# pangsu0613/TransCAR

Hardware: AMD Instinct MI355X
Metric: nuScenes frames/sec (6-cam+radar, 900 queries): fusion decoder (Detr3DHead.forward + box decode), FPN features resident in HBM (higher is better)
Workload: dtype f32 (linear steps and attention core of the batched launches: f16x2 split operands, 3 v_mfma_f32_16x16x32_f16 products, fp32 accumulate; activations of the 32-row tiles held as two f16 planes; 4- / 8-row tiles: f32 MFMA)

## Files before the change

### include/transcar_hip.h

```cpp
#ifndef TRANSCAR_HIP_H
#define TRANSCAR_HIP_H

#include <stddef.h>

#ifdef __cplusplus
extern "C" {
#endif

#define TC_MAX_LEVELS 4
#define TC_MAX_LAYERS 8
#define TC_MAX_RADAR_LAYERS 3
#define TC_MAX_CAM_LOGITS 256
#define TC_ABI_VERSION 13

typedef void* tc_stream_t;

typedef struct { const float* w; const float* b; } tc_linear;
typedef struct { const float* g; const float* b; } tc_lnorm;
typedef struct { tc_linear l0; tc_lnorm n1; tc_linear l3; tc_lnorm n4; } tc_pos_encoder;
typedef struct { tc_linear l0; tc_lnorm n1; tc_linear l3; tc_lnorm n4; tc_linear l6; } tc_cls_branch;
typedef struct { tc_linear l0; tc_linear l2; tc_linear l4; } tc_reg_branch;
typedef struct { tc_linear in_proj; tc_linear out_proj; } tc_mha;

typedef struct {
// ... 196 lines not shown
                       int num_classes, int code_size, int max_num,
                       const float* post_center_range ,
                       float* boxes, float* scores, int* labels, unsigned char* valid,
                       void* workspace, size_t workspace_bytes, tc_stream_t stream);
int tc_box_decode_kept(const float* cls_scores, const float* bbox_preds, int B, int Q, int num_classes,
                       int code_size, int max_num, const float* post_center_range ,
                       float score_threshold, int use_threshold, int z_shift,
                       float* kept_boxes, float* kept_scores, long long* kept_labels, int* kept_count,
                       tc_stream_t stream);

size_t tc_head_workspace_bytes(const tc_head_weights* w, int B, int T);
size_t tc_cam_pregather_workspace_bytes(const tc_head_weights* w, int B);
size_t tc_head_packed_bytes(const tc_head_weights* w);
int tc_head_pack_weights(const tc_head_weights* w, void* packed, size_t packed_bytes,
                         tc_head_weights* packed_view, tc_stream_t stream);
int tc_head_repack_trainable(const tc_head_weights* w, tc_head_weights* packed_view,
                             tc_stream_t stream);
int tc_head_repack_trainable_ex(const tc_head_weights* w, tc_head_weights* packed_view, int copies,
                                tc_stream_t stream);
int tc_head_forward(const tc_head_weights* w, const tc_head_weights* packed_view,
                    const tc_feats_nhwc* feats, int B,
                    const float* lidar2img , float img_h, float img_w,
                    const float* radar_tokens, int T, int pad_mult,
                    float* all_cls_scores, float* all_bbox_preds,
                    const tc_head_aux* aux ,
                    const tc_head_options* options ,
                    void* workspace, size_t workspace_bytes, tc_stream_t stream);



// ... 117 lines not shown
```

### transcar_amd/_lib.py

```python
import ctypes as C
import os

_HERE = os.path.dirname(os.path.abspath(__file__))
LIB_PATH = os.environ.get('TRANSCAR_HIP_LIB') or os.path.join(_HERE, 'lib', 'libtranscar_hip.so')

TC_MAX_LEVELS = 4
TC_MAX_LAYERS = 8
TC_MAX_RADAR_LAYERS = 3
TC_ABI_VERSION = 13

c_fp = C.c_void_p


class TransCARHipError(RuntimeError):
    pass


TC_MAX_CAM_LOGITS = 256


def check_num_points(num_points, num_cams, num_levels):
    if int(num_points) < 1 or num_cams * num_levels * int(num_points) > TC_MAX_CAM_LOGITS:
        raise TransCARHipError(
            'Detr3DCrossAtten(HIP): num_points=%r is not supported (num_points >= 1 and '
# ... 145 lines not shown
    'tc_radar_gated_xattn_fwd': (_i, [_P(tc_mha), _vp, _vp, _vp, _i, _vp, _vp,
                                      _i, _i, _i, _i, _i, _i, _f, _f, _vp,
                                      _vp, _vp, _sz, _vp]),
    'tc_radar_fusion_fwd': (_i, [_P(tc_head_weights), _vp, _vp, _vp, _vp, _i, _i, _i, _i, _i,
                                 _vp, _vp, _vp, _P(tc_head_options), _vp, _sz, _vp]),
    'tc_box_decode_workspace_bytes': (_sz, [_i, _i, _i]),
    'tc_box_decode_topk': (_i, [_vp, _vp, _i, _i, _i, _i, _i, _P(_f), _vp,
                                _vp, _vp, _vp, _vp, _sz, _vp]),
    'tc_box_decode_kept': (_i, [_vp, _vp, _i, _i, _i, _i, _i, _P(_f), _f, _i, _i, _vp, _vp, _vp, _vp, _vp]),
    'tc_head_workspace_bytes': (_sz, [_P(tc_head_weights), _i, _i]),
    'tc_cam_pregather_workspace_bytes': (_sz, [_P(tc_head_weights), _i]),
    'tc_head_packed_bytes': (_sz, [_P(tc_head_weights)]),
    'tc_head_pack_weights': (_i, [_P(tc_head_weights), _vp, _sz,
                                  _P(tc_head_weights), _vp]),
    'tc_head_repack_trainable': (_i, [_P(tc_head_weights), _P(tc_head_weights), _vp]),
    'tc_head_forward': (_i, [_P(tc_head_weights), _P(tc_head_weights),
                             _P(tc_feats_nhwc), _i, _vp,
                             _f, _f, _vp, _i, _i, _vp, _vp, _P(tc_head_aux),
                             _P(tc_head_options), _vp, _sz, _vp]),
    'tc_linear_gated_fwd': (_i, [_vp, _vp, _vp, _vp, _vp, _vp, _i, _i, _i, _vp]),
    'tc_linear_bwd_data': (_i, [_vp, _vp, _vp, _vp, _vp, _vp, _i, _i, _i, _f,
                                _i, _vp]),
    'tc_linear_bwd_weight': (_i, [_vp, _vp, _vp, _vp, _vp, _vp, _i, _i, _i, _f,
                                  _vp]),
    'tc_add_layernorm_bwd': (_i, [_vp, _vp, _vp, _vp, _vp, _vp, _vp, _vp, _i,
                                  _i, _vp]),
    'tc_radar_reference_l1': (_i, [_vp, _P(_f), _vp, _vp, _i, _vp]),
    'tc_box_add_ref_fwd': (_i, [_vp, _i, _vp, _i, _vp, _i, _vp, _i, _vp]),
    'tc_box_add_ref_bwd': (_i, [_vp, _i, _vp, _i, _vp]),
    'tc_radar_attn_core_fwd': (_i, [_vp, _f, _vp, _vp, _i, _vp, _i, _vp, _i,
# ... 79 lines not shown
```

### transcar_amd/csrc/chain.hip

```cpp
#include <stdlib.h>
#include <string.h>

#include <type_traits>

#include "kernels.hpp"
#ifdef TC_CHAIN_STAMPS
__device__ long long g_cam_stamps[4][8];
#define CAM_STAMP(slot)                                                                        \
  do {                                                                                         \
    if (blockIdx.x == 100 && (threadIdx.x & 63) == 0)                                          \
      g_cam_stamps[(threadIdx.x >> 6) & 3][(slot)] = __builtin_amdgcn_s_memtime();             \
  } while (0)
#endif
#include "rowdev.hpp"
#define TC_ONCE_LD(p) ldg4_stream(p)
#ifdef TC_CHAIN_DUMP
__device__ float* g_chain_dump;
__device__ long long g_chain_dump_floats;
#endif

namespace tc {

namespace {

// ... 63 lines not shown
enum Flags : short {
  F_GATE = 1,
  F_SCALEQ = 2,
  F_WOFF = 4,
  F_LN_RELU = 8,
  F_SKIP_NONEXT = 16,
  F_WAVE1 = 32,
  F_NOT_W0 = 64,
  F_LN_XP = 128,
  F_IFHIT = 256,
  F_GPRE = 512,
  F_CMASK = 1024,
  F_CMASK_SCALE = 2048,
  F_CARRY = 4096,
  F_NOT_LAYER0 = 8192,
  F_PRESYNC = 16384
};
enum GSel : short {
  G_NONE = -1, G_HS = 0, G_QK, G_VT, G_INITREF, G_ATTN_O, G_XIN, G_POS, G_CLS, G_KV0, G_KV1, G_KV2,
  G_QF, G_RFEAT, G_COUNT
};

struct StepDesc {
  short kind, wp, wp2, K, N, src, src2, dst, res, act, flags, gsel, gtsel, sync;
};
constexpr StepDesc PROG_DECODER_T[] = {
    {K_LOAD, 0, 0, 0, 0, B_NONE, B_NONE, B_U1, B_NONE, 0, 0, G_ATTN_O, G_NONE, 0},
    {K_LOAD, 0, 0, 0, 0, B_NONE, B_NONE, B_X, B_NONE, 0, 0, G_XIN, G_NONE, 1},
    {K_LINEAR, 1, -1, 256, 256, B_U1, B_NONE, B_U2, B_X, 0, 0, G_NONE, G_NONE, 1},
    {K_LN, 2, -1, 0, 0, B_U2, B_NONE, B_X, B_U1, 0, F_LN_XP, G_NONE, G_NONE, 1},
    {K_LINEAR, 3, -1, 256, N_LOGITS, B_U1, B_NONE, B_L, B_NONE, 0, 0, G_NONE, G_NONE, 0},
    {K_POSENC, 5, 6, 0, 0, B_NONE, B_NONE, B_U2, B_NONE, 0, F_NOT_W0, G_NONE, G_NONE, 1},
    {K_SAMPLE, 0, 0, 0, 0, B_L, B_NONE, B_U3, B_NONE, 0, 0, G_NONE, G_NONE, 1},
    {K_LINEAR, 7, -1, 256, 256, B_U2, B_NONE, B_U1, B_NONE, 0, 0, G_NONE, G_NONE, 1},
    {K_LINEAR, 4, -1, 256, 256, B_U3, B_NONE, B_U2, B_X, 0, 0, G_NONE, G_NONE, 1},
    {K_LN, 9, 8, 0, 0, B_U2, B_U1, B_X, B_NONE, 0, 0, G_NONE, G_NONE, 1},
    {K_LINEAR, 10, -1, 256, 512, B_X, B_NONE, B_A, B_NONE, 1, 0, G_NONE, G_NONE, 1},
    {K_LINEAR, 11, -1, 512, 256, B_A, B_NONE, B_U3, B_X, 0, 0, G_NONE, G_NONE, 1},
    {K_LN, 12, -1, 0, 0, B_U3, B_NONE, B_X, B_U1, 0, F_LN_XP, G_HS, G_NONE, 1},
    {K_LINEAR, 13, -1, 256, 256, B_X, B_NONE, B_U2, B_NONE, 1, 0, G_NONE, G_NONE, 0},
    {K_LINEAR, 16, -1, 256, 512, B_U1, B_NONE, B_NONE, B_NONE, 0, F_SCALEQ | F_SKIP_NONEXT, G_QK, G_NONE, 0},
    {K_LINEAR, 16, -1, 256, 256, B_X, B_NONE, B_NONE, B_NONE, 0, F_WOFF | F_SKIP_NONEXT, G_NONE, G_VT, 1},
    {K_LINEAR, 14, -1, 256, 256, B_U2, B_NONE, B_U3, B_NONE, 1, 0, G_NONE, G_NONE, 0},
    {K_NARROW, 15, -1, 256, N_CODE, B_U3, B_U1, B_L, B_NONE, 0, F_PRESYNC, G_NONE, G_NONE, 1},
    {K_REFUPD, 0, 0, 0, 0, B_L, B_NONE, B_NONE, B_NONE, 0, 0, G_NONE, G_NONE, 0},
    {K_END, 0, 0, 0, 0, 0, 0, 0, 0, 0, 0, 0, 0, 0}};
constexpr StepDesc PROG_PROLOGUE_T[] = {
    {K_LOAD, 0, 0, 0, 0, B_NONE, B_NONE, B_U1, B_NONE, 0, 0, G_POS, G_NONE, 0},
    {K_LOAD, 0, 0, 0, 0, B_NONE, B_NONE, B_X, B_NONE, 0, 0, G_XIN, G_NONE, 1},
    {K_LINEAR, 0, -1, 256, 3, B_U1, B_NONE, B_NONE, B_NONE, 2, 0, G_INITREF, G_NONE, 0},
    {K_LINEAR, 16, -1, 256, 512, B_X, B_U1, B_NONE, B_NONE, 0, F_SCALEQ, G_QK, G_NONE, 0},
    {K_LINEAR, 16, -1, 256, 256, B_X, B_NONE, B_NONE, B_NONE, 0, F_WOFF, G_NONE, G_VT, 0},
    {K_END, 0, 0, 0, 0, 0, 0, 0, 0, 0, 0, 0, 0, 0}};
constexpr StepDesc PROG_RADAR_ENC_T[] = {
    {K_TOKENS, 0, 0, 0, 0, B_NONE, B_NONE, B_A, B_NONE, 0, 0, G_NONE, G_NONE, 1},
    {K_POSENC, 0, 1, 0, 0, B_A, B_NONE, B_U3, B_NONE, 0, 0, G_NONE, G_NONE, 0},
    {K_LINEAR, 4, -1, 36, 64, B_A, B_NONE, B_X, B_NONE, 1, 0, G_NONE, G_NONE, 1},
    {K_LINEAR, 2, -1, 256, 256, B_U3, B_NONE, B_U1, B_NONE, 0, 0, G_NONE, G_NONE, 0},
    {K_LINEAR, 5, -1, 64, 128, B_X, B_NONE, B_U2, B_NONE, 1, 0, G_NONE, G_NONE, 1},
    {K_LINEAR, 6, -1, 128, 256, B_U2, B_NONE, B_X, B_NONE, 1, 0, G_NONE, G_NONE, 1},
    {K_LN, 3, -1, 0, 0, B_U1, B_NONE, B_U2, B_X, 0, F_LN_RELU, G_NONE, G_NONE, 1},
// ... 90 lines not shown
  int last_cls_only;
  const float* ref_in; int ref_mod; float* ref_out; float* box_m;
  CamK cam; unsigned long long* pair_counter;
  const float* pre; const int* premask;
  const float* tokens; int RI, T, pad_mult;
  const float* ref_last; const float* box_in;
  int cen_from_box;
  float rmin[TC_MAX_RADAR_LAYERS], rmax[TC_MAX_RADAR_LAYERS];
  float* all_box; int* hits;
  const int* row_perm;
  float* tape[T_COUNT]; size_t tape_stride; size_t hits_stride;
  DropK rdrop;
  const float* bwd_cxy[TC_MAX_RADAR_LAYERS]; int bwd_ldc[TC_MAX_RADAR_LAYERS];
  const float* bwd_box[TC_MAX_RADAR_LAYERS];
  int* range_status;
  const float* loss_vals;
  float* loss_out;
  const DetAcc* detp;
};
struct ChainK : ChainDev {
  tc_linear pairs[MAX_PAIRS];
  tc_linear gpairs[MAX_PAIRS];
  float* dy[D_COUNT]; size_t dy_stride = 0;
  const float* d_cls = nullptr; const float* d_box = nullptr;
  float* dkv[TC_MAX_RADAR_LAYERS] = {nullptr, nullptr, nullptr};
  size_t w16_delta = 0;
  int npoints = 1;
};

constexpr int table_steps(int prog) {
  return (prog == PROG_DECODER ? (int)(sizeof(PROG_DECODER_T) / sizeof(StepDesc))
          : prog == PROG_PROLOGUE ? (int)(sizeof(PROG_PROLOGUE_T) / sizeof(StepDesc))
          : prog_is_enc_full(prog) ? (int)(sizeof(PROG_RADAR_ENC_T) / sizeof(StepDesc))
          : prog == PROG_RADAR_ENC_A ? (int)(sizeof(PROG_RADAR_ENC_A_T) / sizeof(StepDesc))
          : prog == PROG_RADAR_ENC_B ? (int)(sizeof(PROG_RADAR_ENC_B_T) / sizeof(StepDesc))
          : prog == PROG_RADAR_BWD ? (int)(sizeof(PROG_RADAR_BWD_T) / sizeof(StepDesc))
                                     : (int)(sizeof(PROG_RADAR_LAYER_T) / sizeof(StepDesc))) - 1;
}
constexpr int rec_cap(int prog) { return table_steps(prog) * ((prog_is_radar(prog) || prog == PROG_RADAR_BWD) ? TC_MAX_RADAR_LAYERS : 1); }
static_assert(sizeof(BWD_STORE) / sizeof(short) == table_steps(PROG_RADAR_BWD), "backward maps follow the step table");
static_assert(sizeof(RADAR_TAPE) / sizeof(short) == table_steps(PROG_RADAR) && sizeof(ENC_TAPE) / sizeof(short) == table_steps(PROG_RADAR_ENC),
              "tape maps follow the step tables");
// ... 1107 lines not shown
        const int grow = row_of(row);
        if (j < k.code) S.box[row][j] = k.box_in[(size_t)grow * k.code + j];
        if (j >= 12 && j < 15) {
          const int c = j - 12;
          if (k.cen_from_box) {
            S.cen[row][c] = k.box_in[(size_t)grow * k.code + (c == 2 ? 4 : c)];
          } else {
            const float r = k.ref_last[(size_t)grow * 3 + c];
            const float* pc = k.cam.pc;
            S.cen[row][c] = c < 2 ? __fadd_rn(__fmul_rn(r, pc[3 + c] - pc[c]), pc[c]) : r;
          }
        }
      }
    }
  }
  if constexpr (PROG == PROG_RADAR_BWD) {
    for (int i = threadIdx.x; i < R * LD2; i += NT) (&S.unit[0][0][0])[i] = 0.0f;
    if (threadIdx.x < R * 12) (&S.box[0][0])[threadIdx.x] = 0.0f;
    if (threadIdx.x < R) S.gate[threadIdx.x] = 0;
  }
  __syncthreads();

  START_STAMP(46);
#ifdef TC_CHAIN_STAMPS
  int stamp_i = 0;
  STEP_STAMP();
#endif

  auto do_ln = [&](const StepRes& r) {
    constexpr int NR = R / NW;
    const float* a = buf_ptr(S, r.src); const int lda = buf_ld(r.src);
    const float* c = buf_ptr(S, r.src2); const int ldc = buf_ld(r.src2);
    const bool xp = (r.flags & F_LN_XP) != 0;
    const float* dd = xp ? nullptr : buf_ptr(S, r.res);
    float* dst2 = xp ? buf_ptr(S, r.res) : nullptr;
    float* dst = buf_ptr(S, r.dst);
    float* gdst = r.gd;
    float4 gg, bb;
    if (CHAIN_DBG(k.dbg) & (1 << 17)) {
      gg = make_float4(1.f, 1.f, 1.f, 1.f); bb = make_float4(0.f, 0.f, 0.f, 0.f);
    } else {
      gg = ld4(r.p0 + 4 * lane); bb = ld4(r.p1 + 4 * lane);
    }
    float4 v[NR], pos4[NR];
#pragma unroll
    for (int i = 0; i < NR; ++i) {
      const int row = wave + NW * i;
      pos4[i] = make_float4(0.f, 0.f, 0.f, 0.f);
      if (xp && !(CHAIN_DBG(k.dbg) & (1 << 18))) {
        int prow = min(m0 + row, M - 1);
        if (k.g_mod[G_POS] > 0) prow = prow % k.g_mod[G_POS];
        pos4[i] = ld4(k.g[G_POS] + (size_t)prow * k.g_ld[G_POS] + 4 * lane);
      }
      v[i] = act_ld4<PL>(a + row * lda, 4 * lane);
    }
    if (c != nullptr) {
      const float4 g2 = ld4(r.p2 + 4 * lane), b2 = ld4(r.p3 + 4 * lane);
      float4 cv[NR];
#pragma unroll
      for (int i = 0; i < NR; ++i) cv[i] = act_ld4<PL>(c + (wave + NW * i) * ldc, 4 * lane);
      ln_rows<NR>(cv, g2, b2);
#pragma unroll
      for (int i = 0; i < NR; ++i) v[i] = add4(v[i], relu4(cv[i]));
    }
    ln_rows<NR>(v, gg, bb);
#pragma unroll
    for (int i = 0; i < NR; ++i) {
      const int row = wave + NW * i;
      if (r.flags & F_LN_RELU) v[i] = relu4(v[i]);
// ... 700 lines not shown
    case B_X: return unit0;
    case B_U1: return unit0 + ustride;
    case B_U2: return unit0 + 2 * ustride;
    case B_U3: return unit0 + 3 * ustride;
    case B_L: return (int)(offsetof(Lds, l) / 4);
    default: return -1;
  }
}
template <int R, int PROG>
constexpr size_t chain_lds_bytes() { return sizeof(ChainLds<R, rec_cap(PROG)>); }
inline int buf_ld_h(int id) { return id == B_A ? LD5 : id == B_L ? LDL : LD2; }

template <int R, int PROG, int MM = 0>
void resolve_program(ChainK& k, StepAllT<nw_of(R)>* out) {
  constexpr int NW = nw_of(R);
  const StepDesc* table = prog_table(PROG);
  constexpr int nsteps = table_steps(PROG);
  const int nrep = (prog_is_radar(PROG) || PROG == PROG_RADAR_BWD) ? k.nlayers : 1;
  const int total = nsteps * nrep;
  memset(out, 0, sizeof(StepAllT<NW>) * rec_cap(PROG));
  for (int idx = 0; idx < total; ++idx) {
    const int rep = idx / nsteps, si = idx - rep * nsteps;
    const int layer = PROG == PROG_RADAR_BWD ? k.nlayers - 1 - rep : rep;
    const int pair0 = (prog_is_radar(PROG) || PROG == PROG_RADAR_BWD) ? layer * RADAR_PAIRS : 0;
    const StepDesc d = table[si];
    StepRes& r = out[idx].r;
    r.K = d.K; r.N = d.N;
    r.kind = d.kind; r.src = d.src; r.src2 = d.src2; r.dst = d.dst; r.res = d.res; r.act = d.act;
    r.flags = d.flags; r.sync = d.sync; r.rep = (short)rep; r.si = (short)si;
    if ((d.flags & F_SKIP_NONEXT) && !k.has_next) r.kind = K_NOP;
    if (PROG == PROG_RADAR && k.last_cls_only && rep + 1 < nrep && d.wp >= 6 && d.wp <= 10 &&
        (d.kind == K_LINEAR || d.kind == K_LN || d.kind == K_NARROW))
// ... 263 lines not shown
#endif

void fill_camk(const CamSampleArgs& a, CamK& p);

int launch_prologue(const PrologueArgs& a, hipStream_t s) {
  ChainK k;
  init_k(k);
  k.program = PROG_PROLOGUE; k.M = a.M; k.Q = a.Q; k.has_next = 1; k.w16_delta = a.w16_delta;
  k.pairs[0] = a.refpts; k.pairs[16] = a.in_proj;
  k.g[G_POS] = const_cast<float*>(a.qe); k.g_ld[G_POS] = 512; k.g_mod[G_POS] = a.Q;
  k.g[G_XIN] = const_cast<float*>(a.qe) + 256; k.g_ld[G_XIN] = 512; k.g_mod[G_XIN] = a.Q;
  k.g[G_INITREF] = a.init_ref; k.g_ld[G_INITREF] = 3;
  k.g[G_QK] = a.qk; k.g_ld[G_QK] = 512; k.g[G_VT] = a.vt;
  k.qscale = a.qscale; k.qpad = a.qpad;
  return launch(k, s, "chain(prologue)");
}

static int make_decoder_k(const DecoderChainArgs& a, ChainK& k) {
  TC_REQUIRE(a.code <= 12 && a.cam.num_cams * a.cam.feats.num_levels <= 32, "decoder_chain: code/logit width");
  TC_REQUIRE(a.cam.num_points >= 1 && a.cam.num_cams * a.cam.feats.num_levels * a.cam.num_points <= TC_MAX_CAM_LOGITS,
             "decoder_chain: num_points=%d (num_cams * num_levels * num_points <= %d)", a.cam.num_points, TC_MAX_CAM_LOGITS);
  TC_REQUIRE(a.cam.num_cams <= 8, "decoder_chain: num_cams=%d (<= 8)", a.cam.num_cams);
  for (int l = 0; l < a.cam.feats.num_levels; ++l)
    TC_REQUIRE((long long)a.cam.B * a.cam.num_cams * a.cam.feats.H[l] * a.cam.feats.W[l] < (1ll << 31),
               "decoder_chain: level %d has too many pixels for one call", l);
  init_k(k);
  k.program = PROG_DECODER; k.M = a.M; k.Q = a.Q; k.code = a.code;
  k.nlogits = a.cam.num_cams * a.cam.feats.num_levels * a.cam.num_points;
  k.npoints = a.cam.num_points;
  const tc_decoder_layer& w = *a.w;
// ... 13 lines not shown
  k.g[G_POS] = const_cast<float*>(a.qe); k.g_ld[G_POS] = 512; k.g_mod[G_POS] = a.Q;
  k.g[G_HS] = a.hs; k.g_ld[G_HS] = 256;
  k.g[G_QK] = a.qk; k.g_ld[G_QK] = 512; k.g[G_VT] = a.vt;
  k.qscale = a.qscale; k.qpad = a.qpad;
  k.ref_in = a.ref_in; k.ref_mod = a.ref_mod; k.ref_out = a.ref_out; k.box_m = a.box_m;
  fill_camk(a.cam, k.cam);
  k.pair_counter = a.cam.pair_counter;
  TC_REQUIRE((a.pre == nullptr) == (a.premask == nullptr), "decoder_chain: pre-gathered values and masks come together");
  k.pre = a.pre; k.premask = a.premask;
  TC_REQUIRE(a.tile_rows == 0 || a.tile_rows == 4 || a.tile_rows == 8 || a.tile_rows == 16 || a.tile_rows == 32,
             "decoder_chain: tile_rows=%d (0 = automatic, 4, 8, 16 or 32)", a.tile_rows);
  k.tile_rows = a.tile_rows;
  k.matrix_path = a.matrix_path;
  k.drop = a.drop;
  k.range_status = a.range_status;
  return 0;
}

int launch_decoder_chain(const DecoderChainArgs& a, hipStream_t s) {
  ChainK k;
  int rc = make_decoder_k(a, k);
  if (rc != 0) return rc;
  return launch(k, s, "chain(decoder)");
}

static int make_radar_enc_k(const RadarEncodeArgs& a, ChainK& k, int part = 0) {
  TC_REQUIRE(a.RI <= 64 && (a.RI & 3) == 0, "radar_encode: radar_in_dims=%d", a.RI);
  TC_REQUIRE(a.nlayers == TC_MAX_RADAR_LAYERS, "radar_encode: %d radar layers (3 supported)", a.nlayers);
  init_k(k);
  k.program = part == 1 ? PROG_RADAR_ENC_A : part == 2 ? PROG_RADAR_ENC_B : PROG_RADAR_ENC;
  if (a.tape != nullptr) {
    TC_REQUIRE(part == 0, "radar_encode: the training forward runs the whole encoder program");
    k.program = PROG_RADAR_ENC_TRAIN;
    for (int i = 0; i < T_COUNT; ++i) k.tape[i] = a.tape[i];
  }
  k.M = a.M; k.Q = 1; k.RI = a.RI; k.tokens = a.tokens; k.has_next = 1;
  k.w16_delta = a.w16_delta; k.matrix_path = a.matrix_path; k.range_status = a.range_status;
// ... 227 lines not shown
```

### transcar_amd/csrc/head.hip

```cpp
#include <math.h>
#include <stdarg.h>
#include <stdlib.h>
#include <string.h>

#include "kernels.hpp"

namespace tc {

static thread_local char g_err[512] = "";

void set_error(const char* fmt, ...) {
  va_list ap;
  va_start(ap, fmt);
  vsnprintf(g_err, sizeof(g_err), fmt, ap);
  va_end(ap);
}

int check_launch(const char* what) {
  hipError_t e = hipGetLastError();
  if (e != hipSuccess) {
    set_error("%s: %s", what, hipGetErrorString(e));
    return (int)e;
  }
  return 0;
// ... 56 lines not shown
  const int rows = B * Q;
  const int NL = ncams * feats->num_levels * np;
  TC_TRY(linear(query, C, aw, rows, C, NL, 0, ws.logits, NL, s, pos));
  CamSampleArgs c;
  c.feats = *feats; c.B = B; c.Q = Q; c.C = C; c.num_cams = ncams; c.num_points = np;
  c.lidar2img = l2i; c.ref = ref; c.logits = ws.logits;
  for (int i = 0; i < 6; ++i) c.pc[i] = pc[i];
  c.img_h = img_h; c.img_w = img_w; c.out = ws.sampled; c.vis = nullptr; c.pair_counter = pair_counter;
  TC_TRY(launch_cam_sample(c, s));
  TC_TRY(linear(ws.sampled, C, oproj, rows, C, C, 0, ws.t0, C, s, nullptr, query, C));
  TC_TRY(launch_posenc_l1(ref, 3, 1, pe.l0.w, pe.l0.b, pe.n1.g, pe.n1.b, ws.pe0, rows, s));
  return linear(ws.pe0, C, pe.l3, rows, C, C, 0, ws.pe1, C, s);
}

static int head_points(const tc_head_weights* w) { return w->num_points > 0 ? w->num_points : 1; }

static int check_dims(const tc_head_weights* w) {
  TC_REQUIRE(w != nullptr, "weights pointer is null");
  TC_REQUIRE(w->abi_version == TC_ABI_VERSION, "tc_head_weights.abi_version=%d, library=%d",
             w->abi_version, TC_ABI_VERSION);
  TC_REQUIRE(w->embed_dims == 256 && w->num_heads == 8, "embed_dims=%d num_heads=%d (256/8 supported)",
             w->embed_dims, w->num_heads);
  TC_REQUIRE(w->num_layers >= 1 && w->num_layers <= TC_MAX_LAYERS, "num_layers=%d", w->num_layers);
  TC_REQUIRE(w->num_radar_layers >= 0 && w->num_radar_layers <= TC_MAX_RADAR_LAYERS,
             "num_radar_layers=%d", w->num_radar_layers);
  TC_REQUIRE(w->num_levels == 4, "num_levels=%d (4 supported)", w->num_levels);
  TC_REQUIRE(w->num_points >= 0 && w->num_cams * w->num_levels * head_points(w) <= TC_MAX_CAM_LOGITS,
             "num_points=%d (num_cams * num_levels * num_points <= %d supported)", w->num_points, TC_MAX_CAM_LOGITS);
  TC_REQUIRE((w->ffn_dims & 31) == 0 && (w->radar_in_dims & 3) == 0, "ffn_dims/radar_in_dims alignment");
  return 0;
// ... 28 lines not shown
  h.hs = a.take<float>((size_t)L * rows * C);
  h.reg_tmp = a.take<float>(rows * w->code_size); h.box_m = a.take<float>(rows * w->code_size);
  h.tp0 = a.take<float>(rt * C); h.tp1 = a.take<float>(rt * C);
  h.f0 = a.take<float>(rt * 64); h.f1 = a.take<float>(rt * 128); h.f2 = a.take<float>(rt * C);
  h.radar_feat = a.take<float>(rt * C); h.kv = a.take<float>(rt * 2 * C);
  for (int i = 0; i < TC_MAX_RADAR_LAYERS; ++i) h.kv3[i] = a.take<float>(rt * 2 * C);
  h.qproj = a.take<float>(rows * C); h.rattn = a.take<float>(rows * C);
  h.cxy = a.take<float>(rows * 2); h.addref = a.take<float>(rows * 3);
  h.qf = a.take<float>(rows * C);
  h.hits = a.take<int>((size_t)TC_MAX_RADAR_LAYERS * rows);
  h.perm = a.take<int>(rows); h.hitflag = a.take<int>(rows);
  if (out) *out = h;
  return a.off;
}

static int head_forward_fused(const tc_head_weights* w, const tc_feats_nhwc* feats, int B,
                              const float* lidar2img, float img_h, float img_w,
                              const float* radar_tokens, int T, int pad_mult, float* all_cls_scores,
                              float* all_bbox_preds, const tc_head_aux* aux, const tc_head_options& opt,
                              const HeadWs& h_, hipStream_t s) {
  const int Q = w->num_query, C = w->embed_dims, L = w->num_layers, H = w->num_heads;
  const int code = w->code_size, ncls = w->num_classes;
  const int rows = B * Q, rt = B * T;
  const float attn_qscale = 1.4426950408889634f / sqrtf((float)(C / H));
  HeadWs h = h_;
  if (aux != nullptr) {
    if (aux->inter_states) h.hs = aux->inter_states;
    if (aux->inter_references) h.inter_refs = aux->inter_references;
    if (aux->last_box) h.box_m = aux->last_box;
  }
// ... 10 lines not shown
    for (int r = 0; r < TC_MAX_RADAR_LAYERS; ++r) {
      const tc_mha& m = w->radar[r].attn;
      re.kvproj[r] = tc_linear{m.in_proj.w ? m.in_proj.w + (size_t)C * C : nullptr,
                               m.in_proj.b ? m.in_proj.b + C : nullptr};
      re.kv[r] = h.kv3[r];
    }
    re.radar_feat = h.radar_feat;
    re.w16_delta = w->packed16_delta; re.matrix_path = opt.matrix_path; re.range_status = opt.range_status;
  }

  const bool ddrop = opt.decoder_dropout_p > 0.0f;
  TC_REQUIRE(!ddrop || (unsigned long long)(opt.dropout_seed_stride ? 1 : B) * H * Q * Q < (1ull << 32),
             "decoder dropout: B*H*Q*Q exceeds 32 bits");
  if (radar && ddrop && opt.phase != 1) TC_TRY(launch_radar_encode(re, s));
  const bool folded = !ddrop && w->l0_attn_out != nullptr && w->l0_init_reference != nullptr;
  if (!folded && opt.phase != 2) {
    PrologueArgs pa;
    pa.qe = w->query_embedding; pa.Q = Q; pa.M = rows; pa.refpts = w->reference_points;
    pa.in_proj = w->layers[0].self_attn.in_proj; pa.init_ref = h.init_ref; pa.qk = h.qk; pa.vt = h.vt;
    pa.qpad = h.qpad; pa.qscale = attn_qscale; pa.w16_delta = w->packed16_delta;
    TC_TRY(launch_prologue(pa, s));
  }
  for (int lid = lid_begin; lid < lid_end; ++lid) {
    const bool l0c = folded && lid == 0;
    const float* ref_in = l0c ? w->l0_init_reference
                              : lid == 0 ? h.init_ref : h.inter_refs + (size_t)(lid - 1) * rows * 3;
    DecoderChainArgs d;
    if (ddrop) {
      d.drop = make_drop(opt.decoder_dropout_p, opt.dropout_seed, 16u + 8u * (unsigned)lid, 0u);
      if (opt.dropout_seed_stride != 0) { d.drop.seed_stride = opt.dropout_seed_stride; d.drop.rows_per_sample = (unsigned)Q; }
// ... 22 lines not shown
      if (trows >= 16 && opt.matrix_path != TC_MATRIX_F32) {
        PreGatherArgs pga;
        const bool pre = !ddrop && opt.cam_pregather == 1;
        if (pre) {
          float* pbuf = static_cast<float*>(opt.cam_pregather_ws);
          int* pmask = reinterpret_cast<int*>(pbuf + (size_t)rows * w->num_cams * w->num_levels * C);
          pga.cam = d.cam; pga.M = rows; pga.ref_mod = d.ref_mod; pga.out = pbuf; pga.mask = pmask;
          d.pre = pbuf; d.premask = pmask;
        }
        TC_TRY(launch_self_attn_core_x(h.qk, h.qk + C, 2 * C, h.vt, h.qpad, h.attn_o, C, B, Q, H, s, ddrop ? &d.drop : nullptr,
                                       pre ? &pga : nullptr));
      } else {
        TC_TRY(launch_self_attn_core(h.qk, h.qk + C, 2 * C, h.vt, h.qpad, h.attn_o, C, B, Q, H, s, ddrop ? &d.drop : nullptr));
      }
    }
    if (radar && !ddrop && lid == enc_first) TC_TRY(launch_decoder_chain_with_encoders(d, re, L > 1 ? 1 : 0, s));
    else if (radar && !ddrop && L > 1 && lid == enc_first + 1) TC_TRY(launch_decoder_chain_with_encoders(d, re, 2, s));
    else TC_TRY(launch_decoder_chain(d, s));
  }
  if (opt.phase == 1) return 0;
  if (aux) {
    if (aux->init_reference) {
      if (folded) {
        for (int b = 0; b < B; ++b)
          TC_HIP(hipMemcpyAsync(aux->init_reference + (size_t)b * Q * 3, w->l0_init_reference,
                                (size_t)Q * 3 * 4, hipMemcpyDeviceToDevice, s));
      } else {
        TC_HIP(hipMemcpyAsync(aux->init_reference, h.init_ref, (size_t)rows * 3 * 4, hipMemcpyDeviceToDevice, s));
      }
    }
// ... 405 lines not shown
                       int z_shift, float* kept_boxes, float* kept_scores, long long* kept_labels, int* kept_count,
                       tc_stream_t stream) {
  BoxDecodeKept k{kept_boxes, kept_scores, kept_labels, kept_count, score_threshold, use_threshold, z_shift};
  return launch_box_decode(cls_scores, bbox_preds, B, Q, num_classes, code_size, max_num, post_center_range,
                           nullptr, nullptr, nullptr, nullptr, nullptr, 0, as_stream(stream), &k);
}

size_t tc_head_packed_bytes(const tc_head_weights* w) {
  if (check_dims(w) != 0) return 0;
  tc_head_weights view = *w;
  PackItem items[MAX_PACK_ITEMS];
  const int n = collect_pack_items(w, &view, items);
  size_t total = 0;
  for (int i = 0; i < n; ++i)
    if (!items[i].narrow) total += 3 * arena_slice(packed_floats(items[i].N, items[i].K), 4);
  const size_t Q = w->num_query, C = w->embed_dims, qpad = ((Q + 15) / 16) * 16;
  total += arena_slice(Q * 3, 4) + arena_slice(Q * C, 4) + arena_slice(Q * 2 * C, 4) + arena_slice(C * qpad, 4);
  return total;
}

int tc_head_pack_weights(const tc_head_weights* w, void* packed, size_t packed_bytes,
                         tc_head_weights* packed_view, tc_stream_t stream) {
  TC_TRY(check_dims(w));
  TC_REQUIRE(packed != nullptr && packed_view != nullptr, "pack_weights: null output");
  TC_REQUIRE(packed_bytes >= tc_head_packed_bytes(w), "pack_weights: buffer too small");
  *packed_view = *w;
  PackItem items[MAX_PACK_ITEMS];
  const int n = collect_pack_items(w, packed_view, items);
  Arena a(packed, packed_bytes);
  size_t region_a = 0;
  for (int i = 0; i < n; ++i)
    if (!items[i].narrow) region_a += arena_slice(packed_floats(items[i].N, items[i].K), 4);
  const size_t delta = region_a / sizeof(float);
// ... 16 lines not shown
    float* init_ref = a.take<float>((size_t)Q * 3);
    float* attn_o = a.take<float>((size_t)Q * C);
    float* qk = a.take<float>((size_t)Q * 2 * C);
    float* vt = a.take<float>((size_t)C * qpad);
    hipStream_t s = as_stream(stream);
    TC_HIP(hipMemsetAsync(vt, 0, (size_t)C * qpad * 4, s));
    PrologueArgs pa;
    pa.qe = w->query_embedding; pa.Q = Q; pa.M = Q; pa.refpts = packed_view->reference_points;
    pa.in_proj = packed_view->layers[0].self_attn.in_proj; pa.init_ref = init_ref; pa.qk = qk; pa.vt = vt;
    pa.qpad = qpad; pa.qscale = 1.4426950408889634f / sqrtf((float)(C / H));
    pa.w16_delta = delta;
    TC_TRY(launch_prologue(pa, s));
    TC_TRY(launch_self_attn_core(qk, qk + C, 2 * C, vt, qpad, attn_o, C, 1, Q, H, s));
    packed_view->l0_init_reference = init_ref;
    packed_view->l0_attn_out = attn_o;
  }
  return 0;
}

int tc_head_repack_trainable_ex(const tc_head_weights* w, tc_head_weights* packed_view, int copies,
                                tc_stream_t stream) {
  TC_TRY(check_dims(w));
  TC_REQUIRE(packed_view != nullptr && packed_view->l0_attn_out != nullptr,
             "repack_trainable: packed_view was not produced by tc_head_pack_weights");
  TC_REQUIRE(copies == 1 || copies == 3, "repack_trainable: copies=%d (1: the 4x4x1 copy, 3: both)", copies);
  tc_head_weights scratch = *packed_view;
  PackItem items[MAX_PACK_ITEMS];
  const int n = collect_pack_items(w, &scratch, items);
  const int first = 1 + 10 * w->num_layers;
  PackJob jobs[MAX_PACK_ITEMS];
  int nj = 0;
  for (int i = first; i < n; ++i) {
// ... 292 lines not shown
```

### transcar_amd/csrc/kernels.hpp

```cpp
#pragma once
#include "common.hpp"
#include "../../include/transcar_hip.h"

namespace tc {

struct GemmArgs {
  const float* X = nullptr;  int ldx = 0;
  const float* X2 = nullptr; int x2_cols = 0;
  const float* W = nullptr;  int ldw = 0;
  const float* bias = nullptr;
  const float* R = nullptr;  int ldr = 0;
  const int* rowgate = nullptr;
  float* Y = nullptr;        int ldy = 0;
  float* Yt = nullptr;
  int t_col0 = 0, t_ld = 0, t_rows_per_batch = 1;
  int M = 0, K = 0, N = 0;
  int act = 0;
  float scale = 1.0f; int scale_cols = 0;
};
int launch_gemm(const GemmArgs& a, hipStream_t s);

struct LnArgs {
  const float* a = nullptr;
  const float* b = nullptr;
// ... 49 lines not shown
  int attn_mod = 0, ref_mod = 0;
  const float* x_in; int x_ld, x_mod;
  const float* qe; int Q;
  const float* ref_in; float* ref_out; float* box_m;
  const tc_decoder_layer* w;
  const tc_linear* next_in_proj;
  float qscale;
  float* hs; float* qk; float* vt; int qpad;
  CamSampleArgs cam;
  int code, M;
  int tile_rows = 0;
  int matrix_path = 0;
  DropK drop = DropK{0, 0, 1.0f, 0, 0, 0, 0, 0};
  int* range_status = nullptr;
  const float* pre = nullptr; const int* premask = nullptr;
};
int launch_decoder_chain(const DecoderChainArgs& a, hipStream_t s);

struct RadarEncodeArgs {
  const float* tokens; int RI, M;
  tc_pos_encoder rpe; tc_linear f0, f2, f4;
  int nlayers; tc_linear kvproj[TC_MAX_RADAR_LAYERS]; float* kv[TC_MAX_RADAR_LAYERS];
  float* radar_feat;
  size_t w16_delta = 0;
  float* const* tape = nullptr;
  int matrix_path = 0;
  int* range_status = nullptr;
};
int launch_radar_encode(const RadarEncodeArgs& a, hipStream_t s);
int launch_decoder_chain_with_encoders(const DecoderChainArgs& d, const RadarEncodeArgs& e, int part,
                                       hipStream_t s);

// ... 133 lines not shown
```

Before: 10220.

## Precompute batch-independent layer-0 decoder prefix at weight-pack time

At pack time, the layer-0 decoder steps that depend only on the weights (the residual+LN on the folded self-attention output, the camera-attention logits, the position encoder and the initial reference centres) are run once per tile configuration. The results are stored in the packed arena. At forward time, layer 0 runs a shorter step table that loads these precomputed rows instead of recomputing them per batch row. This moves work out of every forward call, at the cost of extra packed memory and coupling to the pack state, which can be invalidated if weights change without repacking.

```diff
diff --git a/include/transcar_hip.h b/include/transcar_hip.h
--- a/include/transcar_hip.h
+++ b/include/transcar_hip.h
@@ -234,6 +234,7 @@
 size_t tc_head_packed_bytes(const tc_head_weights* w);
 int tc_head_pack_weights(const tc_head_weights* w, void* packed, size_t packed_bytes,
                          tc_head_weights* packed_view, tc_stream_t stream);
+int tc_set_layer0_fold(int on);
 int tc_head_repack_trainable(const tc_head_weights* w, tc_head_weights* packed_view,
                              tc_stream_t stream);
 int tc_head_repack_trainable_ex(const tc_head_weights* w, tc_head_weights* packed_view, int copies,
diff --git a/transcar_amd/_lib.py b/transcar_amd/_lib.py
--- a/transcar_amd/_lib.py
+++ b/transcar_amd/_lib.py
@@ -183,6 +183,7 @@
     'tc_head_pack_weights': (_i, [_P(tc_head_weights), _vp, _sz,
                                   _P(tc_head_weights), _vp]),
     'tc_head_repack_trainable': (_i, [_P(tc_head_weights), _P(tc_head_weights), _vp]),
+    'tc_set_layer0_fold': (_i, [_i]),
     'tc_head_forward': (_i, [_P(tc_head_weights), _P(tc_head_weights),
                              _P(tc_feats_nhwc), _i, _vp,
                              _f, _f, _vp, _i, _i, _vp, _vp, _P(tc_head_aux),
diff --git a/transcar_amd/csrc/chain.hip b/transcar_amd/csrc/chain.hip
--- a/transcar_amd/csrc/chain.hip
+++ b/transcar_amd/csrc/chain.hip
@@ -101,11 +101,14 @@
   F_CMASK_SCALE = 2048,
   F_CARRY = 4096,
   F_NOT_LAYER0 = 8192,
-  F_PRESYNC = 16384
+  F_PRESYNC = 16384,
+  F_LN_CACT = 2
 };
 enum GSel : short {
   G_NONE = -1, G_HS = 0, G_QK, G_VT, G_INITREF, G_ATTN_O, G_XIN, G_POS, G_CLS, G_KV0, G_KV1, G_KV2,
-  G_QF, G_RFEAT, G_COUNT
+  G_QF, G_RFEAT,
+  G_L0X, G_L0POS, G_L0LOG,
+  G_COUNT
 };
 
 struct StepDesc {
@@ -132,6 +135,33 @@
     {K_NARROW, 15, -1, 256, N_CODE, B_U3, B_U1, B_L, B_NONE, 0, F_PRESYNC, G_NONE, G_NONE, 1},
     {K_REFUPD, 0, 0, 0, 0, B_L, B_NONE, B_NONE, B_NONE, 0, 0, G_NONE, G_NONE, 0},
     {K_END, 0, 0, 0, 0, 0, 0, 0, 0, 0, 0, 0, 0, 0}};
+constexpr StepDesc PROG_DECODER_PREFIX_T[] = {
+    {K_LOAD, 0, 0, 0, 0, B_NONE, B_NONE, B_U1, B_NONE, 0, 0, G_ATTN_O, G_NONE, 0},
+    {K_LOAD, 0, 0, 0, 0, B_NONE, B_NONE, B_X, B_NONE, 0, 0, G_XIN, G_NONE, 1},
+    {K_LINEAR, 1, -1, 256, 256, B_U1, B_NONE, B_U2, B_X, 0, 0, G_NONE, G_NONE, 1},
+    {K_LN, 2, -1, 0, 0, B_U2, B_NONE, B_X, B_U1, 0, F_LN_XP, G_L0X, G_NONE, 1},
+    {K_LINEAR, 3, -1, 256, N_LOGITS, B_U1, B_NONE, B_L, B_NONE, 0, 0, G_L0LOG, G_NONE, 0},
+    {K_POSENC, 5, 6, 0, 0, B_NONE, B_NONE, B_U2, B_NONE, 0, F_NOT_W0, G_NONE, G_NONE, 1},
+    {K_LINEAR, 7, -1, 256, 256, B_U2, B_NONE, B_U1, B_NONE, 0, 0, G_NONE, G_NONE, 1},
+    {K_LN, 8, -1, 0, 0, B_U1, B_NONE, B_U2, B_NONE, 0, F_LN_RELU, G_L0POS, G_NONE, 1},
+    {K_END, 0, 0, 0, 0, 0, 0, 0, 0, 0, 0, 0, 0, 0}};
+constexpr StepDesc PROG_DECODER_L0_T[] = {
+    {K_LOAD, 0, 0, 0, 0, B_NONE, B_NONE, B_X, B_NONE, 0, 0, G_L0X, G_NONE, 1},
+    {K_SAMPLE, 0, 0, 0, 0, B_L, B_NONE, B_U3, B_NONE, 0, 0, G_NONE, G_NONE, 1},
+    {K_LINEAR, 4, -1, 256, 256, B_U3, B_NONE, B_U2, B_X, 0, 0, G_NONE, G_NONE, 1},
+    {K_LN, 9, -1, 0, 0, B_U2, B_NONE, B_X, B_NONE, 0, F_LN_CACT, G_NONE, G_L0POS, 1},
+    {K_LINEAR, 10, -1, 256, 512, B_X, B_NONE, B_A, B_NONE, 1, 0, G_NONE, G_NONE, 1},
+    {K_LINEAR, 11, -1, 512, 256, B_A, B_NONE, B_U3, B_X, 0, 0, G_NONE, G_NONE, 1},
+    {K_LN, 12, -1, 0, 0, B_U3, B_NONE, B_X, B_U1, 0, F_LN_XP, G_HS, G_NONE, 1},
+    {K_LINEAR, 13, -1, 256, 256, B_X, B_NONE, B_U2, B_NONE, 1, 0, G_NONE, G_NONE, 0},
+    {K_LINEAR, 16, -1, 256, 512, B_U1, B_NONE, B_NONE, B_NONE, 0, F_SCALEQ | F_SKIP_NONEXT, G_QK, G_NONE, 0},
+    {K_LINEAR, 16, -1, 256, 256, B_X, B_NONE, B_NONE, B_NONE, 0, F_WOFF | F_SKIP_NONEXT, G_NONE, G_VT, 1},
+    {K_LINEAR, 14, -1, 256, 256, B_U2, B_NONE, B_U3, B_NONE, 1, 0, G_NONE, G_NONE, 0},
+    {K_NARROW, 15, -1, 256, N_CODE, B_U3, B_U1, B_L, B_NONE, 0, F_PRESYNC, G_NONE, G_NONE, 1},
+    {K_REFUPD, 0, 0, 0, 0, B_L, B_NONE, B_NONE, B_NONE, 0, 0, G_NONE, G_NONE, 0},
+    {K_END, 0, 0, 0, 0, 0, 0, 0, 0, 0, 0, 0, 0, 0}};
+static_assert(sizeof(PROG_DECODER_PREFIX_T) <= sizeof(PROG_DECODER_T) && sizeof(PROG_DECODER_L0_T) <= sizeof(PROG_DECODER_T),
+              "the layer-0 tables fit the decoder program's records");
 constexpr StepDesc PROG_PROLOGUE_T[] = {
     {K_LOAD, 0, 0, 0, 0, B_NONE, B_NONE, B_U1, B_NONE, 0, 0, G_POS, G_NONE, 0},
     {K_LOAD, 0, 0, 0, 0, B_NONE, B_NONE, B_X, B_NONE, 0, 0, G_XIN, G_NONE, 1},
@@ -252,6 +282,9 @@
   const float* bwd_cxy[TC_MAX_RADAR_LAYERS]; int bwd_ldc[TC_MAX_RADAR_LAYERS];
   const float* bwd_box[TC_MAX_RADAR_LAYERS];
   int* range_status;
+  const int* l0_range;
+  const float* l0_cen;
+  const float* l0_logits;
   const float* loss_vals;
   float* loss_out;
   const DetAcc* detp;
@@ -264,6 +297,7 @@
   float* dkv[TC_MAX_RADAR_LAYERS] = {nullptr, nullptr, nullptr};
   size_t w16_delta = 0;
   int npoints = 1;
+  const StepDesc* table = nullptr; int table_n = 0;
 };
 
 constexpr int table_steps(int prog) {
@@ -1401,6 +1435,23 @@
       }
     }
   }
+  if constexpr (PROG == PROG_DECODER) {
+    if (k.l0_cen != nullptr && threadIdx.x < 3 * R) {
+      const int row = threadIdx.x / 3, c = threadIdx.x - 3 * row;
+      S.cen[row][c] = k.l0_cen[(size_t)(min(m0 + row, M - 1) % k.Q) * 3 + c];
+    }
+    if (k.l0_logits != nullptr && 4 * lane < k.nlogits) {
+      for (int row = wave; row < R; row += NW) {
+        const float4 v = ld4(k.l0_logits + (size_t)(min(m0 + row, M - 1) % k.Q) * k.nlogits + 4 * lane);
+        if constexpr (MP) act_st4<PL>(&S.unit[3][row][0], 4 * lane, v);
+        else *reinterpret_cast<float4*>(&S.l[row][4 * lane]) = v;
+      }
+    }
+  }
+  if constexpr (PROG == PROG_DECODER && MM == 1) {
+    if (k.l0_range != nullptr && k.range_status != nullptr && block == 0 && threadIdx.x == 0 && *k.l0_range != 0)
+      atomicOr(k.range_status, 1);
+  }
   if constexpr (PROG == PROG_RADAR_BWD) {
     for (int i = threadIdx.x; i < R * LD2; i += NT) (&S.unit[0][0][0])[i] = 0.0f;
     if (threadIdx.x < R * 12) (&S.box[0][0])[threadIdx.x] = 0.0f;
@@ -1419,6 +1470,7 @@
     const float* a = buf_ptr(S, r.src); const int lda = buf_ld(r.src);
     const float* c = buf_ptr(S, r.src2); const int ldc = buf_ld(r.src2);
     const bool xp = (r.flags & F_LN_XP) != 0;
+    const bool ca = PROG == PROG_DECODER && (r.flags & F_LN_CACT) != 0;
     const float* dd = xp ? nullptr : buf_ptr(S, r.res);
     float* dst2 = xp ? buf_ptr(S, r.res) : nullptr;
     float* dst = buf_ptr(S, r.dst);
@@ -1438,8 +1490,14 @@
         int prow = min(m0 + row, M - 1);
         if (k.g_mod[G_POS] > 0) prow = prow % k.g_mod[G_POS];
         pos4[i] = ld4(k.g[G_POS] + (size_t)prow * k.g_ld[G_POS] + 4 * lane);
+      } else if (ca) {
+        pos4[i] = ld4(r.gt + (size_t)(min(m0 + row, M - 1) % k.Q) * 256 + 4 * lane);
       }
       v[i] = act_ld4<PL>(a + row * lda, 4 * lane);
+    }
+    if (ca) {
+#pragma unroll
+      for (int i = 0; i < NR; ++i) v[i] = add4(v[i], pos4[i]);
     }
     if (c != nullptr) {
       const float4 g2 = ld4(r.p2 + 4 * lane), b2 = ld4(r.p3 + 4 * lane);
@@ -2170,8 +2228,9 @@
 template <int R, int PROG, int MM = 0>
 void resolve_program(ChainK& k, StepAllT<nw_of(R)>* out) {
   constexpr int NW = nw_of(R);
-  const StepDesc* table = prog_table(PROG);
-  constexpr int nsteps = table_steps(PROG);
+  const bool own = PROG == PROG_DECODER && k.table != nullptr;
+  const StepDesc* table = own ? k.table : prog_table(PROG);
+  const int nsteps = own ? k.table_n : table_steps(PROG);
   const int nrep = (prog_is_radar(PROG) || PROG == PROG_RADAR_BWD) ? k.nlayers : 1;
   const int total = nsteps * nrep;
   memset(out, 0, sizeof(StepAllT<NW>) * rec_cap(PROG));
@@ -2465,6 +2524,21 @@
   k.g[G_QK] = a.qk; k.g_ld[G_QK] = 512; k.g[G_VT] = a.vt;
   k.qscale = a.qscale; k.qpad = a.qpad;
   return launch(k, s, "chain(prologue)");
+}
+
+struct L0Fold { float *x, *pos, *logits, *cen; int* range; };
+constexpr int L0_FOLD_SLOTS = 5;
+static size_t l0_fold_slot_bytes(int Q) {
+  return 2 * arena_slice((size_t)Q * 256, 4) + arena_slice((size_t)Q * TC_MAX_CAM_LOGITS, 4) + arena_slice((size_t)Q * 3, 4) +
+         arena_slice(1, 4);
+}
+static L0Fold l0_fold_slot(void* base, int Q, int rows, bool f16x2) {
+  const int slot = rows == 4 ? 0 : rows == 8 ? 1 : rows == 16 ? (f16x2 ? 3 : 2) : 4;
+  Arena a(static_cast<char*>(base) + slot * l0_fold_slot_bytes(Q), l0_fold_slot_bytes(Q));
+  L0Fold f;
+  f.x = a.take<float>((size_t)Q * 256); f.pos = a.take<float>((size_t)Q * 256);
+  f.logits = a.take<float>((size_t)Q * TC_MAX_CAM_LOGITS); f.cen = a.take<float>((size_t)Q * 3); f.range = a.take<int>(1);
+  return f;
 }
 
 static int make_decoder_k(const DecoderChainArgs& a, ChainK& k) {
@@ -2508,13 +2582,41 @@
   k.matrix_path = a.matrix_path;
   k.drop = a.drop;
   k.range_status = a.range_status;
+  if (a.l0_fold != nullptr) {
+    TC_REQUIRE(a.drop.thr == 0 && a.pre == nullptr, "decoder_chain: the folded layer 0 is an eval-mode layer that gathers for itself");
+    const L0Fold f = l0_fold_slot(a.l0_fold, a.Q, tile_rows(k), use_f16x2(k));
+    const int Q = a.Q;
+    k.g[G_L0X] = f.x; k.g_ld[G_L0X] = 256; k.g_mod[G_L0X] = Q;
+    k.g[G_L0POS] = f.pos; k.g_ld[G_L0POS] = 256; k.g_mod[G_L0POS] = Q;
+    k.g[G_L0LOG] = f.logits; k.g_ld[G_L0LOG] = k.nlogits; k.g_mod[G_L0LOG] = Q;
+    if (a.l0_fold_prefix) {
+      TC_REQUIRE(a.M == Q, "decoder_chain: the layer-0 prefix runs on the Q query rows");
+      k.table = PROG_DECODER_PREFIX_T; k.table_n = (int)(sizeof(PROG_DECODER_PREFIX_T) / sizeof(StepDesc)) - 1;
+      k.range_status = f.range;
+    } else {
+      k.table = PROG_DECODER_L0_T; k.table_n = (int)(sizeof(PROG_DECODER_L0_T) / sizeof(StepDesc)) - 1;
+      k.l0_range = f.range; k.l0_cen = f.cen; k.l0_logits = f.logits;
+    }
+  }
   return 0;
+}
+
+size_t l0_fold_bytes(int Q) { return L0_FOLD_SLOTS * l0_fold_slot_bytes(Q); }
+
+__global__ void l0_centres_kernel(const float* ref, float* cen, int n) {
+  const int i = blockIdx.x * blockDim.x + threadIdx.x;
+  if (i < n) cen[i] = inverse_sigmoidf_(ref[i]);
 }
 
 int launch_decoder_chain(const DecoderChainArgs& a, hipStream_t s) {
   ChainK k;
   int rc = make_decoder_k(a, k);
   if (rc != 0) return rc;
+  if (a.l0_fold != nullptr && a.l0_fold_prefix) {
+    const L0Fold f = l0_fold_slot(a.l0_fold, a.Q, tile_rows(k), use_f16x2(k));
+    hipLaunchKernelGGL(l0_centres_kernel, dim3((3 * a.Q + 255) / 256), dim3(256), 0, s, a.ref_in, f.cen, 3 * a.Q);
+    if (int e = check_launch("l0_centres")) return e;
+  }
   return launch(k, s, "chain(decoder)");
 }
 
diff --git a/transcar_amd/csrc/head.hip b/transcar_amd/csrc/head.hip
--- a/transcar_amd/csrc/head.hip
+++ b/transcar_amd/csrc/head.hip
@@ -2,6 +2,9 @@
 #include <stdarg.h>
 #include <stdlib.h>
 #include <string.h>
+
+#include <mutex>
+#include <vector>
 
 #include "kernels.hpp"
 
@@ -94,6 +97,7 @@
 }
 
 static int head_points(const tc_head_weights* w) { return w->num_points > 0 ? w->num_points : 1; }
+static int head_logits(const tc_head_weights* w) { return w->num_cams * w->num_levels * head_points(w); }
 
 static int check_dims(const tc_head_weights* w) {
   TC_REQUIRE(w != nullptr, "weights pointer is null");
@@ -152,6 +156,31 @@
   return a.off;
 }
 
+static std::mutex g_fold_mu;
+static bool g_fold_on = true;
+static std::vector<const void*> g_unfolded;
+static void note_arena_fold(const void* l0_attn_out, bool folded) {
+  std::lock_guard<std::mutex> g(g_fold_mu);
+  for (size_t i = 0; i < g_unfolded.size(); ++i)
+    if (g_unfolded[i] == l0_attn_out) { g_unfolded.erase(g_unfolded.begin() + i); break; }
+  if (!folded) g_unfolded.push_back(l0_attn_out);
+}
+static bool arena_folded(const void* l0_attn_out) {
+  std::lock_guard<std::mutex> g(g_fold_mu);
+  for (const void* p : g_unfolded)
+    if (p == l0_attn_out) return false;
+  return true;
+}
+static size_t l0_consts_bytes(const tc_head_weights* w) {
+  const size_t Q = w->num_query, C = w->embed_dims, qpad = ((Q + 15) / 16) * 16;
+  return arena_slice(Q * 3, 4) + arena_slice(Q * C, 4) + arena_slice(Q * 2 * C, 4) + arena_slice(C * qpad, 4);
+}
+static void* l0_fold_block(const tc_head_weights* v) {
+  const size_t Q = v->num_query, C = v->embed_dims, qpad = ((Q + 15) / 16) * 16;
+  return const_cast<char*>(reinterpret_cast<const char*>(v->l0_attn_out)) + arena_slice(Q * C, 4) +
+         arena_slice(Q * 2 * C, 4) + arena_slice(C * qpad, 4);
+}
+
 static int head_forward_fused(const tc_head_weights* w, const tc_feats_nhwc* feats, int B,
                               const float* lidar2img, float img_h, float img_w,
                               const float* radar_tokens, int T, int pad_mult, float* all_cls_scores,
@@ -192,6 +221,7 @@
              "decoder dropout: B*H*Q*Q exceeds 32 bits");
   if (radar && ddrop && opt.phase != 1) TC_TRY(launch_radar_encode(re, s));
   const bool folded = !ddrop && w->l0_attn_out != nullptr && w->l0_init_reference != nullptr;
+  void* l0_fold = folded && arena_folded(w->l0_attn_out) ? l0_fold_block(w) : nullptr;
   if (!folded && opt.phase != 2) {
     PrologueArgs pa;
     pa.qe = w->query_embedding; pa.Q = Q; pa.M = rows; pa.refpts = w->reference_points;
@@ -244,6 +274,7 @@
         TC_TRY(launch_self_attn_core(h.qk, h.qk + C, 2 * C, h.vt, h.qpad, h.attn_o, C, B, Q, H, s, ddrop ? &d.drop : nullptr));
       }
     }
+    if (l0c) d.l0_fold = l0_fold;
     if (radar && !ddrop && lid == enc_first) TC_TRY(launch_decoder_chain_with_encoders(d, re, L > 1 ? 1 : 0, s));
     else if (radar && !ddrop && L > 1 && lid == enc_first + 1) TC_TRY(launch_decoder_chain_with_encoders(d, re, 2, s));
     else TC_TRY(launch_decoder_chain(d, s));
@@ -679,9 +710,7 @@
   size_t total = 0;
   for (int i = 0; i < n; ++i)
     if (!items[i].narrow) total += 3 * arena_slice(packed_floats(items[i].N, items[i].K), 4);
-  const size_t Q = w->num_query, C = w->embed_dims, qpad = ((Q + 15) / 16) * 16;
-  total += arena_slice(Q * 3, 4) + arena_slice(Q * C, 4) + arena_slice(Q * 2 * C, 4) + arena_slice(C * qpad, 4);
-  return total;
+  return total + l0_consts_bytes(w) + l0_fold_bytes(w->num_query);
 }
 
 int tc_head_pack_weights(const tc_head_weights* w, void* packed, size_t packed_bytes,
@@ -728,8 +757,45 @@
     TC_TRY(launch_self_attn_core(qk, qk + C, 2 * C, vt, qpad, attn_o, C, 1, Q, H, s));
     packed_view->l0_init_reference = init_ref;
     packed_view->l0_attn_out = attn_o;
+    void* fold = a.take<char>(l0_fold_bytes(Q));
+    bool fold_on;
+    { std::lock_guard<std::mutex> g(g_fold_mu); fold_on = g_fold_on; }
+    if (fold_on) {
+      TC_HIP(hipMemsetAsync(fold, 0, l0_fold_bytes(Q), s));
+      static const int rows_mm[5][2] = {{4, TC_MATRIX_F32}, {8, TC_MATRIX_F32}, {16, TC_MATRIX_F32}, {16, TC_MATRIX_F16X2},
+                                        {32, TC_MATRIX_F16X2}};
+      tc_feats_nhwc nofeats;
+      memset(&nofeats, 0, sizeof(nofeats));
+      nofeats.num_levels = w->num_levels;
+      for (const auto& rm : rows_mm) {
+        DecoderChainArgs d;
+        d.attn_o = attn_o; d.attn_mod = Q; d.ref_mod = Q;
+        d.x_in = w->query_embedding + C; d.x_ld = 2 * C; d.x_mod = Q;
+        d.qe = w->query_embedding; d.Q = Q;
+        d.ref_in = init_ref; d.ref_out = nullptr; d.box_m = nullptr;
+        d.w = &packed_view->layers[0]; d.next_in_proj = nullptr;
+        d.qscale = 1.4426950408889634f / sqrtf((float)(C / H));
+        d.hs = nullptr; d.qk = nullptr; d.vt = nullptr; d.qpad = qpad;
+        d.cam.feats = nofeats; d.cam.B = 1; d.cam.Q = Q; d.cam.C = C; d.cam.num_cams = w->num_cams;
+        d.cam.num_points = head_points(w);
+        d.cam.lidar2img = nullptr; d.cam.ref = init_ref; d.cam.logits = nullptr;
+        for (int i = 0; i < 6; ++i) d.cam.pc[i] = w->pc_range[i];
+        d.cam.img_h = 1.0f; d.cam.img_w = 1.0f; d.cam.out = nullptr; d.cam.vis = nullptr; d.cam.pair_counter = nullptr;
+        d.code = w->code_size; d.M = Q; d.tile_rows = rm[0]; d.matrix_path = rm[1];
+        d.l0_fold = fold; d.l0_fold_prefix = 1;
+        TC_TRY(launch_decoder_chain(d, s));
+      }
+    }
+    note_arena_fold(attn_o, fold_on);
   }
   return 0;
+}
+
+int tc_set_layer0_fold(int on) {
+  std::lock_guard<std::mutex> g(g_fold_mu);
+  const int was = g_fold_on ? 1 : 0;
+  g_fold_on = on != 0;
+  return was;
 }
 
 int tc_head_repack_trainable_ex(const tc_head_weights* w, tc_head_weights* packed_view, int copies,
diff --git a/transcar_amd/csrc/kernels.hpp b/transcar_amd/csrc/kernels.hpp
--- a/transcar_amd/csrc/kernels.hpp
+++ b/transcar_amd/csrc/kernels.hpp
@@ -87,8 +87,10 @@
   DropK drop = DropK{0, 0, 1.0f, 0, 0, 0, 0, 0};
   int* range_status = nullptr;
   const float* pre = nullptr; const int* premask = nullptr;
+  void* l0_fold = nullptr; int l0_fold_prefix = 0;
 };
 int launch_decoder_chain(const DecoderChainArgs& a, hipStream_t s);
+size_t l0_fold_bytes(int Q);
 
 struct RadarEncodeArgs {
   const float* tokens; int RI, M;
```

After: 10400, median of 6. +1.7%, better.
